# td-kwj-zp2023/webgpu-msm-twisted-edwards

Hardware: AMD Instinct MI355X
Metric: MSMs/sec at n=2^20 Twisted-Edwards BLS12 (pipelined throughput = 1000/ms_per_step; single-MSM latency in latency_ms) (higher is better)
Workload: dtype u32

## Files before the change

### webgpu-msm-twisted-edwards_amd/csrc/kernels.hip.hpp

```cpp
#pragma once
#include <hip/hip_runtime.h>
#include "curve.hpp"

namespace te {

#define TE_BATCH_MAX 8
struct batch_ptrs { const uint4* p[TE_BATCH_MAX]; };
struct batch_slabs { uint32_t s[TE_BATCH_MAX]; };

struct digits_params {
  uint32_t half[10];
  uint32_t zero_digit;
  uint32_t sc_stride;
  uint32_t n, nst;
  int num_windows;
  int w_first, w_step, nw_local;
  uint32_t half_code, logS, P, CH, chunk_len;
};

struct pnt_slot { uint4 q[8]; };
__device__ __forceinline__ void prep_points_block(uint32_t blk, uint4* __restrict__ lds, const uint4* __restrict__ pts, pnt_slot* __restrict__ recs, uint32_t n) {
  const uint32_t t = threadIdx.x, base = blk * 256u;
  const bool active = t < 256u;
  const uint32_t pieces_in = (n - base < 256u ? n - base : 256u) * 4u;
  const uint4* __restrict__ src = pts + (size_t)base * 4u;
  if (active) {
#pragma unroll
    for (int j = 0; j < 4; j++) {
      const uint32_t g = (uint32_t)j * 256u + t;
      lds[g] = src[g < pieces_in ? g : 0u];
    }
  }
  __syncthreads();
  uint4 a0 = make_uint4(0u, 0u, 0u, 0u), a1 = a0, b0 = a0, b1 = a0;
  if (active) { a0 = lds[4 * t + 0]; a1 = lds[4 * t + 1]; b0 = lds[4 * t + 2]; b1 = lds[4 * t + 3]; }
// ... 519 lines not shown
  __syncthreads();
  const uint32_t c0 = cnt_s[t];
  const size_t gb = (size_t)k * g.B + (size_t)p * g.S + t;
  if (!single) {
    if (c0) atomicAdd(&a.bucket_count[gb], c0);
    wait_own_accesses();
    __syncthreads();
    if (t == 0) pj[2] = (handoff_arrive(&a.part_ticket[k * g.P + p]) + 1u == (cntp + TE_L2_CAP - 1u) / TE_L2_CAP) ? 1u : 0u;
    __syncthreads();
    if (pj[2]) (void)seg_plan_block(p, k, t < g.S ? ld_agent(a.bucket_count + gb) : 0u, g, a.pa, PL, pb, cntp, sbp);
    return;
  }
  if (t < g.S) a.bucket_count[gb] = c0;
  const uint32_t ex = seg_plan_block(p, k, c0, g, a.pa, PL, pb, cntp, sbp);
  if (t < g.S) a.pa.bucket_cursor[gb] = pb + ex + c0;
  off_s[t] = ex;
  __syncthreads();
#pragma unroll
  for (int c = 0; c < 5; c++) {
    uint32_t kv[8], iv[8]; piece_group<PK>(r, c, kv, iv);
    const uint32_t e0 = ((uint32_t)c * 256u + t) * 8u;
#pragma unroll
    for (int e = 0; e < 8; e++) {
      const uint32_t pos = e0 + (uint32_t)e;
      if (pos >= head && pos < total) list[atomicAdd(&off_s[kv[e] & 0x7fffu], 1u)] = iv[e] | ((kv[e] >> 15) << 31);
    }
  }
  __syncthreads();
  uint32_t* out = a.sorted + (size_t)k * g.n + pb;
  for (uint32_t s = t; s < cntp; s += 256u) out[s] = list[s];
}

#define TE_ORDER_REGS 32u
__device__ __forceinline__ void order_scatter_block(uint32_t ob, uint32_t nob, uint32_t* __restrict__ lds, const uint32_t* __restrict__ lenv, uint32_t ids,
                                                    const uint32_t* __restrict__ size_hist, uint32_t* __restrict__ rel_cursor,
                                                    uint32_t* __restrict__ order, uint32_t* __restrict__ num_segments, uint32_t max_len) {
  uint32_t* const h = lds; uint32_t* const base = lds + 1024; uint32_t* const sm = lds + 2048;
  const uint32_t per = (ids + nob - 1) / nob;
  const uint32_t lo = min(ids, ob * per), hi = min(ids, lo + per);
  const bool in_regs = per <= TE_ORDER_REGS * 256u;
  uint32_t lv[TE_ORDER_REGS];
  if (in_regs) {
#pragma unroll
    for (uint32_t j = 0; j < TE_ORDER_REGS; j++) { const uint32_t g = lo + j * 256u + threadIdx.x; lv[j] = g < hi ? lenv[g] : TE_SEG_INVALID; }
  }
  for (uint32_t j = threadIdx.x; j < 1024u; j += 256u) h[j] = 0;
  {
    uint32_t run = 0;
    for (uint32_t c = (1023u - min(max_len, 1023u)) >> 8; c < 4u; c++) {
      const uint32_t s = 1023u - (c * 256u + threadIdx.x);
      uint32_t part[TE_HIST_COPIES];
#pragma unroll
      for (uint32_t r = 0; r < TE_HIST_COPIES; r++) part[r] = size_hist[r * 1024u + s];
      uint32_t cnt_s = 0;
#pragma unroll
      for (uint32_t r = 0; r < TE_HIST_COPIES; r++) cnt_s += part[r];
      uint32_t bt;
      const uint32_t ex = block_excl_scan(cnt_s, sm, bt);
      base[s] = run + ex;
      run += bt;
    }
    if (ob == 0 && threadIdx.x == 0) *num_segments = run;
  }
  __syncthreads();
  if (in_regs) {
#pragma unroll
    for (uint32_t j = 0; j < TE_ORDER_REGS; j++) if (lv[j] != TE_SEG_INVALID) atomicAdd(&h[min(lv[j], 1023u)], 1u);
  } else {
    for (uint32_t g = lo + threadIdx.x; g < hi; g += 256u) { const uint32_t l = lenv[g]; if (l != TE_SEG_INVALID) atomicAdd(&h[min(l, 1023u)], 1u); }
  }
  __syncthreads();
  for (uint32_t j = threadIdx.x; j < 1024u; j += 256u) { base[j] += h[j] ? atomicAdd(&rel_cursor[j], h[j]) : 0u; h[j] = 0; }
  __syncthreads();
  if (in_regs) {
#pragma unroll
    for (uint32_t j = 0; j < TE_ORDER_REGS; j++) {
      if (lv[j] == TE_SEG_INVALID) continue;
      const uint32_t sz = min(lv[j], 1023u);
      order[base[sz] + atomicAdd(&h[sz], 1u)] = lo + j * 256u + threadIdx.x;
    }
  } else {
    for (uint32_t g = lo + threadIdx.x; g < hi; g += 256u) {
      const uint32_t l = lenv[g];
      if (l == TE_SEG_INVALID) continue;
      const uint32_t sz = min(l, 1023u);
      order[base[sz] + atomicAdd(&h[sz], 1u)] = g;
    }
  }
}

#define TE_PLACE_LDS_WORDS (4u * 256u + TE_L2_LIST + TE_L2_LIST / 4u + 2u + 17u)
template <bool PK>
__device__ __forceinline__ void l2_place_piece(uint32_t p, uint32_t k, uint32_t a0, uint32_t b0, uint32_t* __restrict__ lds,
                                               const uint16_t* __restrict__ part_keys, const uint32_t* __restrict__ part_idx,
                                               uint32_t* __restrict__ bucket_cursor, uint32_t* __restrict__ sorted, const sort_geom& g) {
  uint32_t* const cnt_s = lds; uint32_t* const lex_s = lds + 256; uint32_t* const off_s = lds + 512; uint32_t* const gbase_s = lds + 768;
  uint32_t* const list = lds + 1024;
  uint8_t* const list_b = reinterpret_cast<uint8_t*>(list + TE_L2_LIST);
  uint32_t* const sm = list + TE_L2_LIST + TE_L2_LIST / 4u + 2u;
  const uint32_t t = threadIdx.x, len = b0 - a0;
  const uint16_t* keys_row = part_keys + (size_t)k * g.nst; const uint32_t* idx_row = part_idx + (size_t)k * g.nst;
  uint32_t* out = sorted + (size_t)k * g.n;
  cnt_s[t] = 0u;
  __syncthreads();
  piece_regs r; uint32_t head, total;
  load_piece<PK>(keys_row, idx_row, a0, b0, t, true, r, head, total);
#pragma unroll
  for (int c = 0; c < 5; c++) {
    uint32_t kv[8], iv[8]; piece_group<PK>(r, c, kv, iv);
    const uint32_t e0 = ((uint32_t)c * 256u + t) * 8u;
#pragma unroll
    for (int e = 0; e < 8; e++) { const uint32_t pos = e0 + (uint32_t)e; if (pos >= head && pos < total) atomicAdd(&cnt_s[kv[e] & 0x7fffu], 1u); }
  }
  __syncthreads();
  wave0_excl_scan(cnt_s, lex_s, 256u, &sm[16]);
  {
    const uint32_t c0 = cnt_s[t];
    gbase_s[t] = c0 ? atomicAdd(&bucket_cursor[(size_t)k * g.B + (size_t)p * g.S + t], c0) : 0u;
  }
  __syncthreads();
  off_s[t] = lex_s[t];
  gbase_s[t] -= lex_s[t];
  __syncthreads();
#pragma unroll
  for (int c = 0; c < 5; c++) {
    uint32_t kv[8], iv[8]; piece_group<PK>(r, c, kv, iv);
    const uint32_t e0 = ((uint32_t)c * 256u + t) * 8u;
#pragma unroll
    for (int e = 0; e < 8; e++) {
      const uint32_t pos = e0 + (uint32_t)e;
      if (pos >= head && pos < total) {
        const uint32_t b = kv[e] & 0x7fffu;
        const uint32_t slot = atomicAdd(&off_s[b], 1u);
        list[slot] = iv[e] | ((kv[e] >> 15) << 31); list_b[slot] = (uint8_t)b;
      }
    }
  }
  __syncthreads();
  for (uint32_t s = t; s < len; s += 256u) out[gbase_s[list_b[s]] + s] = list[s];
}

struct order_args { const uint32_t* lenv; uint32_t ids; const uint32_t* size_hist; uint32_t* rel_cursor; uint32_t* order; uint32_t* num_segments; uint32_t order_cols, max_len; };
template <bool PK>
__global__ void __launch_bounds__(256, TE_L2_WAVES) k_l2_place_order(const uint16_t* __restrict__ part_keys, const uint32_t* __restrict__ part_idx,
                                                           const uint32_t* __restrict__ part_start, const uint32_t* __restrict__ part_count,
                                                           uint32_t* __restrict__ bucket_cursor, uint32_t* __restrict__ sorted, sort_geom g, order_args oa) {
  __shared__ uint32_t lds[TE_PLACE_LDS_WORDS];
  if (blockIdx.x < oa.order_cols) {
    order_scatter_block(blockIdx.y * oa.order_cols + blockIdx.x, gridDim.y * oa.order_cols, lds, oa.lenv, oa.ids, oa.size_hist, oa.rel_cursor, oa.order, oa.num_segments, oa.max_len);
    return;
  }
  const uint32_t k = gridDim.y - 1u - blockIdx.y;
  const uint32_t px = blockIdx.x - oa.order_cols, extra = gridDim.x - oa.order_cols - g.P, bx = px < extra ? g.P + px : px - extra;
  const uint32_t* pc = part_count + k * g.P;
  uint32_t p, j;
  if (!l2_piece_of_block(bx, pc, g.P, bx < g.P ? 0u : part_count[gridDim.y * g.P + k], lds, lds + 32, p, j)) return;
  const uint32_t cntp = pc[p], pb = part_start[k * g.P + p];
  if (cntp <= TE_L2_CAP) return;
  const uint32_t a0 = pb + j * TE_L2_CAP;
  l2_place_piece<PK>(p, k, a0, min(pb + cntp, a0 + TE_L2_CAP), lds, part_keys, part_idx, bucket_cursor, sorted, g);
}

template <int N> struct geo {
  static constexpr uint32_t PW = 4u * N;
  static constexpr uint32_t PQ = PW / 4u;
  static constexpr uint32_t RW = N == 9 ? 27u : 4u * N;
  static constexpr uint32_t SQ = N == 9 ? 8u : N;
  static constexpr uint32_t LQ = (RW + 3u) / 4u;
};
template <int N> struct rec_slot { uint4 q[geo<N>::SQ]; };
static_assert(sizeof(rec_slot<9>) == sizeof(pnt_slot) && sizeof(rec_slot<14>) == 224, "record slots");

template <int N> __device__ __forceinline__ pnt_t<N> load_pnt(const rec_slot<N>* __restrict__ recs, uint32_t entry) {
  const uint4* q = recs[entry & 0x7fffffffu].q;
  constexpr uint32_t LQ = geo<N>::LQ;
  uint4 u[LQ];
#pragma unroll
  for (uint32_t j = 0; j < LQ; j++) u[j] = q[j];
  uint32_t w[4 * LQ];
#pragma unroll
  for (uint32_t j = 0; j < LQ; j++) { w[4 * j] = u[j].x; w[4 * j + 1] = u[j].y; w[4 * j + 2] = u[j].z; w[4 * j + 3] = u[j].w; }
  pnt_t<N> r;
// ... 47 lines not shown
#pragma unroll
  for (int j = 0; j < 10; j++) u[j] = reinterpret_cast<const u4a8*>(base)[j];
  const u2a8 t = *reinterpret_cast<const u2a8*>(base + 40);
  uint32_t w[42];
#pragma unroll
  for (int j = 0; j < 10; j++) { w[4 * j] = u[j].v[0]; w[4 * j + 1] = u[j].v[1]; w[4 * j + 2] = u[j].v[2]; w[4 * j + 3] = u[j].v[3]; }
  w[40] = t.v[0]; w[41] = t.v[1];
  pnt_aff377 r;
#pragma unroll
  for (int j = 0; j < 14; j++) { r.hm.v[j] = w[j]; r.hp.v[j] = w[14 + j]; r.dt.v[j] = w[28 + j]; }
  return r;
}
__device__ __forceinline__ void store_pnt_aff377(rec_aff377* dst, const pnt_aff377& r) {
#pragma unroll
  for (int j = 0; j < 14; j++) { dst->w[j] = r.hm.v[j]; dst->w[14 + j] = r.hp.v[j]; dst->w[28 + j] = r.dt.v[j]; }
}
template <int N, int RK> struct rec_kind;
template <int N> struct rec_kind<N, 0> {
  using slot = rec_slot<N>; using pnt = pnt_t<N>;
  static __device__ __forceinline__ pnt load(const slot* __restrict__ recs, uint32_t e) { return load_pnt<N>(recs, e); }
};
template <> struct rec_kind<14, 1> {
  using slot = rec_aff377; using pnt = pnt_aff377;
  static __device__ __forceinline__ pnt load(const slot* __restrict__ recs, uint32_t e) { return load_pnt_aff377(recs, e); }
};

struct __attribute__((aligned(4))) idx4 { uint32_t v[4]; };
#define TE_CLK_SLOTS 64u
#define TE_IDX_STRIP 16u
template <int N, int RK = 0>
__global__ void __launch_bounds__(256, N == 9 ? 3 : 2) k_accumulate(const typename rec_kind<N, RK>::slot* __restrict__ recs, const uint32_t* __restrict__ sorted,
                                                    const uint32_t* __restrict__ bucket_start, const uint32_t* __restrict__ bucket_count,
                                                    const uint32_t* __restrict__ seg_base, const uint32_t* __restrict__ seg_bucket,
                                                    const uint32_t* __restrict__ seg_lenv, const uint32_t* __restrict__ order,
                                                    const uint32_t* __restrict__ num_segments, ete_t<N>* __restrict__ buckets,
                                                    ete_t<N>* __restrict__ seg_out, uint32_t n, uint32_t logB, uint32_t seg_len, uint32_t ids, uint32_t onto,
                                                    uint32_t win_per_msm, batch_slabs slabs, unsigned long long* __restrict__ clk) {
  __shared__ uint32_t idx_strip[256 * TE_IDX_STRIP];
  using RT = rec_kind<N, RK>; using P = typename RT::pnt;
#if defined(TE_ACC_TWO_WAVES)
  if constexpr (N == 9) asm volatile("" ::: "v175");
#endif
  unsigned long long* const slot = clk ? clk + (blockIdx.x & (TE_CLK_SLOTS - 1u)) : nullptr;
  const unsigned long long t0_wall = clk ? (unsigned long long)wall_clock64() : 0ull, t0_core = clk ? (unsigned long long)clock64() : 0ull;
  if (clk && threadIdx.x == 0) atomicMax(slot, ~t0_wall);
  const uint32_t gid = blockIdx.x * 256u + threadIdx.x;
  if (gid >= (order ? *num_segments : ids)) return;
  const uint32_t sgm = order ? order[gid] : gid;
  const uint32_t g = seg_bucket[sgm];
  if (g == TE_SEG_INVALID) return;
  const uint32_t k = g >> logB;
  recs += (size_t)slabs.s[k / win_per_msm] * n;
  const uint32_t part = sgm - seg_base[g];
  const uint32_t cnt = seg_lenv[sgm];
  const uint32_t* lst = sorted + (size_t)k * n + bucket_start[g] + part * seg_len;
  ete_t<N> acc = (onto && part == 0u) ? load_ete<N>(buckets + g) : ete_identity_t<N>();
  if (cnt) {
    const uint32_t last = cnt - 1u;
    uint32_t j0 = 0;
    uint32_t e = lst[0], e_n = lst[min(1u, last)];
    P cur = RT::load(recs, e);
    if (!(onto && part == 0u)) {
      const P first = pnt_cneg(cur, (e >> 31) != 0u);
      e = e_n; e_n = lst[min(2u, last)];
      cur = RT::load(recs, e);
      acc = ete_from_pnt(first);
      j0 = 1;
    }
    uint32_t* const strip = idx_strip + threadIdx.x * TE_IDX_STRIP;
    auto refill = [&](uint32_t pos) {
      const idx4* src = reinterpret_cast<const idx4*>(lst + pos);
      idx4* dst = reinterpret_cast<idx4*>(strip);
#pragma unroll
      for (uint32_t h = 0; h < TE_IDX_STRIP / 4u; h += 2u) {
        const idx4 v0 = src[h], v1 = src[h + 1u];
        dst[h] = v0; dst[h + 1u] = v1;
      }
    };
    if (((j0 + 2u) & (TE_IDX_STRIP - 1u)) != 0u) refill((j0 + 2u) & ~(TE_IDX_STRIP - 1u));
    for (uint32_t j = j0; j < cnt; j++) {
      const uint32_t e_cur = e;
      P nxt = cur;
      const uint32_t pn = j + 2u;
      if ((pn & (TE_IDX_STRIP - 1u)) == 0u) refill(pn);
      const uint32_t e_nn = strip[pn & (TE_IDX_STRIP - 1u)];
      if (j + 1 < cnt) { e = e_n; nxt = RT::load(recs, e); }
      acc = ete_madd(acc, pnt_cneg(cur, (e_cur >> 31) != 0u));
      cur = nxt; e_n = e_nn;
    }
  }
  const bool whole = bucket_count[g] <= seg_len;
  store_ete<N>(whole ? buckets + g : seg_out + sgm, acc);
  if (clk && (uint32_t)__lane_id() == (uint32_t)__ffsll((long long)__ballot(1)) - 1u) {
    const unsigned long long t1_wall = (unsigned long long)wall_clock64(), t1_core = (unsigned long long)clock64();
    atomicMax(slot + TE_CLK_SLOTS, t1_wall);
    atomicAdd(slot + 2u * TE_CLK_SLOTS, t1_core - t0_core); atomicAdd(slot + 3u * TE_CLK_SLOTS, t1_wall - t0_wall);
  }
}

template <int N> struct sum_job_t {
  const ete_t<N>* in; ete_t<N>* out;
  uint32_t n_out;
  uint32_t K, inner;
  uint32_t in_per_window, out_per_window;
};
template <int N> struct sum_jobs_t { sum_job_t<N> j[4]; };
template <int N> __device__ __forceinline__ ete_t<N> pair_swap(const ete_t<N>& a) {
  ete_t<N> r;
#pragma unroll
  for (int i = 0; i < N; i++) {
    r.x.v[i] = (uint32_t)__builtin_amdgcn_mov_dpp((int)a.x.v[i], 0xb1, 0xf, 0xf, true);
    r.y.v[i] = (uint32_t)__builtin_amdgcn_mov_dpp((int)a.y.v[i], 0xb1, 0xf, 0xf, true);
    r.z.v[i] = (uint32_t)__builtin_amdgcn_mov_dpp((int)a.z.v[i], 0xb1, 0xf, 0xf, true);
    r.t.v[i] = (uint32_t)__builtin_amdgcn_mov_dpp((int)a.t.v[i], 0xb1, 0xf, 0xf, true);
  }
  return r;
}
template <int N, bool PAIR>
__global__ void __launch_bounds__(256, N == 9 ? 2 : 1) k_sum_groups(sum_jobs_t<N> js, uint32_t nw) {
  const sum_job_t<N>& j = js.j[blockIdx.y];
  constexpr uint32_t TPO = PAIR ? 2u : 1u;
  const uint32_t total = j.n_out * nw * TPO, Kt = j.K / TPO;
  for (uint32_t gt = blockIdx.x * 256u + threadIdx.x; gt < total; gt += gridDim.x * 256u) {
    const uint32_t g = gt / TPO, half = gt % TPO;
    const uint32_t k = g / j.n_out, o = g - k * j.n_out;
// ... 511 lines not shown
```

### webgpu-msm-twisted-edwards_amd/csrc/te_msm.hip

```cpp
#include <hip/hip_runtime.h>
#include <stdint.h>
#include <stdio.h>
#include <stdlib.h>
#include <string.h>
#include <string>
#include <vector>
#include <deque>
#include <algorithm>
#include <functional>
#include <chrono>
#include <thread>
#include <mutex>
#include <condition_variable>
#include <memory>
#if defined(__x86_64__)
#include <immintrin.h>
#endif

#include "../../include/te_msm.h"
#include "host_tail.hpp"
#include "synth.hpp"
#include "kernels.hip.hpp"
#include "check.hip.hpp"
#include "from_x.hip.hpp"
// ... 18 lines not shown
                                            : curve_sizes{TE_MSM_POINT_BYTES, TE_MSM_SCALAR_BYTES, sizeof(te::ete), sizeof(te::rec_slot<9>), TE_MSM_PARTIAL_BYTES, 64};
}
inline size_t rec_bytes_of(int curve, int rec_kind) { return (curve == TE_MSM_CURVE_BLS12_377_G1 && rec_kind == 1) ? sizeof(te::rec_aff377) : sizes_of(curve).rec; }
static_assert(TE377_TAIL_ROW_BYTES == TE_MSM_PARTIAL_BYTES_BLS12_377 && sizeof(te::ete_t<14>) * 5 == TE377_TAIL_ROW_BYTES, "row layout");
constexpr size_t TE_MAX_ROW_BYTES = TE377_TAIL_ROW_BYTES;

struct plan_t {
  int curve = 0;
  int c = 0, W = 0, nw = 0;
  int nw1 = 0, batch = 1;
  int w_first = 0, w_step = 1;
  uint32_t B = 0, logB = 0;
  int signed_digits = 1;
  uint32_t dw[4] = {0, 0, 0, 0};
  uint32_t CH = 0, chunk_len = 0, nst = 0;
  uint32_t seg_len = 64;
  uint32_t S = 0, logS = 0, P = 0;
  uint32_t packed = 0;
  int rec_kind = 0;
  int fb_rb = 0, fb_c = 0, fb_W = 0;
};

struct workset_t {
  hipStream_t stream = nullptr, copy_stream = nullptr;
  int hw_queue_class = -1;
  hipEvent_t ev_copy = nullptr, ev_start = nullptr;
  size_t cap[40] = {};
  uint8_t* d_recs = nullptr;
  uint16_t *d_digits = nullptr, *d_part_keys = nullptr;
  uint32_t *d_counts1 = nullptr, *d_part_start = nullptr, *d_part_count = nullptr, *d_part_idx = nullptr, *d_seg_part_base = nullptr;
  uint32_t *d_bucket_count = nullptr, *d_bucket_start = nullptr, *d_bucket_cursor = nullptr, *d_sorted = nullptr;
  uint32_t *d_seg_base = nullptr, *d_seg_bucket = nullptr, *d_seg_lenv = nullptr, *d_order = nullptr;
  uint32_t *d_split_list = nullptr, *d_chunk_list = nullptr;
  uint8_t *d_seg_out = nullptr, *d_buckets = nullptr, *d_red[4] = {};
  uint32_t *d_zero = nullptr; size_t zero_words = 0;
  size_t zero_clean_words = 0;
  uint32_t *d_err = nullptr, *d_num_seg = nullptr, *d_size_hist = nullptr, *d_size_cursor = nullptr;
  uint32_t* d_part_ticket = nullptr;
  uint8_t* d_partials = nullptr;
  uint32_t* h_err = nullptr;
  uint8_t* h_partials = nullptr;
  uint32_t* h_err_dev = nullptr;
  bool rows_on_host = false;
  hipEvent_t ev_done = nullptr;
  hipEvent_t ev_result = nullptr;
  hipEvent_t ev[ST_COUNT + 1] = {};
  plan_t plan; uint64_t n = 0; bool used = false;
  te_sched::slot_t slot;
  std::string job_err;
  int prof_level = 0;
  hipStream_t last_stream = nullptr;
  void *d_in_points = nullptr, *d_in_scalars = nullptr; size_t cap_in_points = 0, cap_in_scalars = 0;
  std::vector<hipEvent_t> piece_events;
  uint8_t* h_ring = nullptr; std::vector<hipEvent_t> ring_ev; size_t ring_next = 0;
  uint64_t idle_calls = 0;
  uint32_t* d_fb_remap = nullptr;
  uint32_t* d_fb_fill = nullptr;
  const void* fb_scalars = nullptr; uint64_t fb_n = 0;
  int slab = -1;
  bool slab_run = false;
  const uint8_t* recs_last = nullptr;
  te_bases* bound = nullptr;
  int pt_rc = 0; int64_t pt_index = -1; int pt_reason = 0;
  uint8_t* d_batch_rows = nullptr;
  uint32_t* d_in_idx = nullptr;
};
// ... 164 lines not shown

template <typename T> int ensure(te_ctx* ctx, workset_t& ws, T*& ptr, size_t& cap_bytes, size_t need_elems) {
  const size_t need = need_elems * sizeof(T);
  if (ptr && need <= cap_bytes) return 0;
  if (ptr) HIP_TRY(ctx, hipFree(ptr));
  ptr = nullptr; cap_bytes = 0;
  HIP_TRY(ctx, hipMalloc((void**)&ptr, need ? need : 16));
  cap_bytes = need;
  return 0;
}

int ensure_buffers(te_ctx* ctx, gpu_t& d, workset_t& ws, uint64_t n, const plan_t& p, bool need_recs = true) {
  HIP_TRY(ctx, hipSetDevice(d.device));
  const size_t nd = (size_t)p.nw * p.nst + 64, wb = (size_t)p.nw * p.B, ab = sizes_of(p.curve).acc;
  int rc = 0;
  if (need_recs && (rc = ensure(ctx, ws, ws.d_recs, ws.cap[0], (size_t)n * sizes_of(p.curve).rec * (size_t)p.batch))) return rc;
  if ((rc = ensure(ctx, ws, ws.d_digits, ws.cap[1], nd))) return rc;
  if ((rc = ensure(ctx, ws, ws.d_sorted, ws.cap[2], nd))) return rc;
  {
    const size_t c1 = (size_t)p.nw * p.CH * p.P;
    ws.zero_words = Z_END + c1 + wb + (size_t)p.nw * p.P + 64;
    { const uint32_t* before = ws.d_zero; if ((rc = ensure(ctx, ws, ws.d_zero, ws.cap[3], ws.zero_words))) return rc; if (ws.d_zero != before) ws.zero_clean_words = 0; }
    ws.d_err = ws.d_zero; ws.d_num_seg = ws.d_zero + Z_KEEP; ws.d_size_hist = ws.d_zero + Z_HIST; ws.d_size_cursor = ws.d_zero + Z_CURSOR;
    ws.d_partials = reinterpret_cast<uint8_t*>(ws.d_zero + Z_ROWS);
    ws.d_counts1 = ws.d_zero + Z_END; ws.d_bucket_count = ws.d_counts1 + c1; ws.d_part_ticket = ws.d_bucket_count + wb;
    ws.d_fb_fill = ws.d_part_ticket + (size_t)p.nw * p.P;
  }
  if (p.fb_rb && (rc = ensure(ctx, ws, ws.d_fb_remap, ws.cap[27], nd))) return rc;
  if ((rc = ensure(ctx, ws, ws.d_bucket_start, ws.cap[5], wb))) return rc;
  if ((rc = ensure(ctx, ws, ws.d_bucket_cursor, ws.cap[16], wb))) return rc;
  if ((rc = ensure(ctx, ws, ws.d_seg_part_base, ws.cap[17], (size_t)p.nw * p.P))) return rc;
  const size_t smax = wb + (size_t)p.nw * (n / (uint64_t)p.seg_len) + 16;
  if ((rc = ensure(ctx, ws, ws.d_order, ws.cap[7], smax))) return rc;
  if ((rc = ensure(ctx, ws, ws.d_seg_bucket, ws.cap[20], smax))) return rc;
  if ((rc = ensure(ctx, ws, ws.d_seg_lenv, ws.cap[21], smax))) return rc;
  if ((rc = ensure(ctx, ws, ws.d_seg_out, ws.cap[22], smax * ab))) return rc;
  if ((rc = ensure(ctx, ws, ws.d_seg_base, ws.cap[23], wb + 1))) return rc;
  if ((rc = ensure(ctx, ws, ws.d_split_list, ws.cap[24], wb + 1))) return rc;
  if ((rc = ensure(ctx, ws, ws.d_chunk_list, ws.cap[26], 2 * (wb + smax / TE_GIANT_RUN + 2)))) return rc;
  if ((rc = ensure(ctx, ws, ws.d_part_start, ws.cap[6], (size_t)p.nw * p.P))) return rc;
  if ((rc = ensure(ctx, ws, ws.d_buckets, ws.cap[8], wb * ab))) return rc;
  if ((rc = ensure(ctx, ws, ws.d_part_count, ws.cap[9], (size_t)p.nw * p.P + (size_t)p.nw))) return rc;
  if ((rc = ensure(ctx, ws, ws.d_part_keys, ws.cap[14], p.packed ? 8 : nd))) return rc;
  if ((rc = ensure(ctx, ws, ws.d_part_idx, ws.cap[15], nd))) return rc;
  if ((rc = ensure(ctx, ws, ws.d_red[0], ws.cap[10], (wb / 2 + 1) * ab))) return rc;
  if ((rc = ensure(ctx, ws, ws.d_red[1], ws.cap[11], (wb / 4 + 1) * ab))) return rc;
  if ((rc = ensure(ctx, ws, ws.d_red[2], ws.cap[12], (wb / 2 + 1) * ab))) return rc;
  if ((rc = ensure(ctx, ws, ws.d_red[3], ws.cap[13], (wb / 4 + 1) * ab))) return rc;
  return 0;
}

template <int C> void launch_digits(const te::batch_ptrs& sc, int batch, uint16_t* dg, const te::digits_params& prm, uint32_t* err, uint32_t* counts1, hipStream_t s) {
  hipLaunchKernelGGL(te::k_digits<C>, dim3((prm.nst + TE_DIG_BLOCK - 1u) / TE_DIG_BLOCK, batch), dim3(TE_DIG_THREADS), 0, s, sc, dg, prm, err, counts1);
}
static_assert(TE_BATCH_MAX == TE_MSM_MAX_BATCH, "batch tables");
template <int C> void launch_digits_ragged(const void* sc, const te::ragged_tab& tab, int batch, uint16_t* dg, const te::digits_params& prm, uint32_t* err, uint32_t* counts1, hipStream_t s) {
  hipLaunchKernelGGL(te::k_digits_ragged<C>, dim3((prm.nst + TE_DIG_BLOCK - 1u) / TE_DIG_BLOCK, batch), dim3(TE_DIG_THREADS), 0, s, static_cast<const uint4*>(sc), tab, dg, prm, err, counts1);
}
static_assert(TE_RAGGED_MAX == TE_BATCH_SEQ_MAX && TE_BATCH_SEQ_MAX == TE_MSM_BATCH_SEQ_MAX, "ragged tables");

struct msm_launch {
  te_ctx* ctx; workset_t& ws; plan_t p;
  const void* d_points; const void* d_scalars; uint64_t n; void* d_partials_out;
  int prof;
  hipStream_t stream;
  bool own_rows = false;
// ... 123 lines not shown
          const uint32_t per_row = (n32 + 511u) / 512u;
          hipLaunchKernelGGL(te::k_part_scatter_prep377, dim3(sblocks + rows * per_row), dim3(512), 0, stream, sa, sblocks, tab, row_slab,
                             reinterpret_cast<te::rec_slot<14>*>(recs_out()), n32, per_row, rows * per_row);
        } else {
          const uint32_t per_row = (n32 + 255u) / 256u;
          hipLaunchKernelGGL(te::k_part_scatter_prep, dim3(sblocks + rows * per_row), dim3(512), 0, stream, sa, sblocks, tab, row_slab,
                             reinterpret_cast<te::pnt_slot*>(recs_out()), n32, per_row, rows * per_row);
        }
      } else if (idx) {
        hipLaunchKernelGGL(te::k_part_scatter_indexed, dim3(p.CH, p.nw), dim3(512), 0, stream, sa, te::index_args{idx, idx_count, idx_pos, ws.d_err});
      } else {
        hipLaunchKernelGGL(te::k_part_scatter, dim3(p.CH, p.nw), dim3(512), 0, stream, sa);
      }
    }
    mark(ST_BSORT);
    if (p.nw > 0) {
      const uint32_t l2_blocks = p.P + n32 / TE_L2_CAP + 1u;
      te::l2_args la;
      la.part_keys = ws.d_part_keys; la.part_idx = ws.d_part_idx; la.part_start = ws.d_part_start; la.part_count = ws.d_part_count;
      la.bucket_count = ws.d_bucket_count; la.sorted = ws.d_sorted; la.part_ticket = ws.d_part_ticket; la.g = sg;
      la.pa.part_start = ws.d_part_start; la.pa.part_count = ws.d_part_count; la.pa.seg_part_base = ws.d_seg_part_base;
      la.pa.bucket_start = ws.d_bucket_start; la.pa.bucket_cursor = ws.d_bucket_cursor; la.pa.seg_base = ws.d_seg_base; la.pa.seg_bucket = ws.d_seg_bucket;
      la.pa.seg_lenv = ws.d_seg_lenv; la.pa.size_hist = ws.d_size_hist; la.pa.split_list = ws.d_split_list; la.pa.split_count = ws.d_num_seg + 1;
      la.pa.chunk_list = ws.d_chunk_list; la.pa.seg_len = p.seg_len; la.pa.cap_w = cap_w; la.pa.chunk_cap = chunk_cap();
      if (p.packed) hipLaunchKernelGGL(te::k_l2_local<true>, dim3(l2_blocks, p.nw), dim3(256), 0, stream, la);
      else hipLaunchKernelGGL(te::k_l2_local<false>, dim3(l2_blocks, p.nw), dim3(256), 0, stream, la);
      te::order_args oa;
      oa.lenv = ws.d_seg_lenv; oa.ids = smax(); oa.size_hist = ws.d_size_hist; oa.rel_cursor = ws.d_size_cursor; oa.order = ws.d_order; oa.num_segments = ws.d_num_seg;
      {
        const uint32_t by_regs = (smax() + TE_ORDER_REGS * 256u * (uint32_t)p.nw - 1u) / (TE_ORDER_REGS * 256u * (uint32_t)p.nw);
        oa.order_cols = std::min(64u, std::max(by_regs, (uint32_t)std::max(1, 128 / p.nw)));
      }
      oa.max_len = std::min(p.seg_len, 1023u);
      if (p.packed)
        hipLaunchKernelGGL(te::k_l2_place_order<true>, dim3(oa.order_cols + l2_blocks, p.nw), dim3(256), 0, stream, ws.d_part_keys, ws.d_part_idx, ws.d_part_start,
                           ws.d_part_count, ws.d_bucket_cursor, ws.d_sorted, sg, oa);
      else
        hipLaunchKernelGGL(te::k_l2_place_order<false>, dim3(oa.order_cols + l2_blocks, p.nw), dim3(256), 0, stream, ws.d_part_keys, ws.d_part_idx, ws.d_part_start,
                           ws.d_part_count, ws.d_bucket_cursor, ws.d_sorted, sg, oa);
    }
    mark(ST_ORDER);
    return 0;
  }

  bool bls() const { return p.curve == TE_MSM_CURVE_BLS12_377_G1; }

  template <int N, int RK> int accumulate_t() {
    mark(ST_ACCUM);
    if (p.nw > 0) {
      const uint32_t n32 = this->n32(), smax = this->smax();
      const uint32_t* order = ctx->opt_sort ? ws.d_order : nullptr;
      using slot_t = typename te::rec_kind<N, RK>::slot;
      hipLaunchKernelGGL((te::k_accumulate<N, RK>), dim3((smax + 255) / 256), dim3(256), 0, stream, reinterpret_cast<const slot_t*>(bound ? bound : recs_out()), ws.d_sorted,
                         ws.d_bucket_start, ws.d_bucket_count, ws.d_seg_base, ws.d_seg_bucket, ws.d_seg_lenv, order, ws.d_num_seg,
                         reinterpret_cast<te::ete_t<N>*>(ws.d_buckets), reinterpret_cast<te::ete_t<N>*>(ws.d_seg_out), n32, p.logB, p.seg_len, smax, onto ? 1u : 0u,
                         ragged ? (uint32_t)p.nw : (uint32_t)p.nw1, ragged ? te::batch_slabs{} : slabs(),
                         prof ? reinterpret_cast<unsigned long long*>(ws.d_zero + Z_CLOCK) : nullptr);
    }
    return 0;
  }
  int accumulate() { return bls() ? (p.rec_kind == 1 ? accumulate_t<14, 1>() : accumulate_t<14, 0>()) : accumulate_t<9, 0>(); }

  template <int N> int combine_t() {
    if (p.nw <= 0) return 0;
    using E = te::ete_t<N>;
    hipLaunchKernelGGL(te::k_seg_combine_all<N>, dim3(256 + 1024), dim3(256), 0, stream, ws.d_split_list, ws.d_num_seg + 1, ws.d_chunk_list,
                       ws.d_bucket_count, ws.d_seg_base, reinterpret_cast<E*>(ws.d_seg_out), reinterpret_cast<E*>(ws.d_buckets), p.seg_len, chunk_cap(), 256u,
                       ws.d_bucket_start, ws.d_bucket_cursor);
    return 0;
  }
  int combine() { return bls() ? combine_t<14>() : combine_t<9>(); }

  template <int N> int reduce_t() {
    if (p.nw > 0) {
      using E = te::ete_t<N>;
      const uint32_t w0 = p.dw[0], w1 = p.dw[1], w2 = p.dw[2], w3 = p.dw[3];
      const uint32_t L = 1u << (w0 + w1), H = 1u << (w2 + w3);
      struct chain_t { const E* cur; uint32_t n, r; E* buf[2]; int pp; };
      E* const bk = reinterpret_cast<E*>(ws.d_buckets);
      chain_t ch[2] = {{bk, p.B, L, {reinterpret_cast<E*>(ws.d_red[0]), reinterpret_cast<E*>(ws.d_red[1])}, 0},
                       {bk, p.B, H, {reinterpret_cast<E*>(ws.d_red[2]), reinterpret_cast<E*>(ws.d_red[3])}, 0}};
      for (;;) {
        te::sum_jobs_t<N> js; memset(&js, 0, sizeof js);
        uint32_t most = 0; int nj = 0;
        for (int i = 0; i < 2; i++) {
          chain_t& c = ch[i];
          if (c.r <= 4u) continue;
// ... 305 lines not shown
  HIP_TRY(ctx, hipEventRecord(ws.ev_done, stream));
  return 0;
}

int collect_stage_ms(te_ctx* ctx, const gpu_t& d, workset_t& ws) {
  if (!ws.prof_level) return 0;
  bool ok = true;
  for (int i = 0; i < ST_COUNT; i++) {
    float ms = -1.0f;
    if (ws.prof_level >= 2 || i == ST_ACCUM) ok = ok && hipEventElapsedTime(&ms, ws.ev[i], ws.ev[i + 1]) == hipSuccess;
    ctx->stage_ms[i] = ms;
  }
  {
    uint64_t raw[4 * TE_CLK_SLOTS]; memcpy(raw, ws.h_err + Z_CLOCK, sizeof raw);
    uint64_t c[4] = {0, 0, 0, 0};
    for (uint32_t i = 0; i < TE_CLK_SLOTS; i++) {
      c[0] = std::max(c[0], raw[i]); c[1] = std::max(c[1], raw[TE_CLK_SLOTS + i]);
      c[2] += raw[2 * TE_CLK_SLOTS + i]; c[3] += raw[3 * TE_CLK_SLOTS + i];
    }
    const int khz = d.wall_clock_khz;
    const bool have = c[0] && c[1] && khz > 0 && c[1] > ~c[0];
    const double ms = have ? (double)(c[1] - ~c[0]) / khz : -1.0;
    ctx->stage_ms[ST_COUNT] = (float)ms;
    ctx->stage_ms[ST_COUNT + 1] = (have && c[2] && c[3]) ? (float)((double)c[2] / (double)c[3] * khz * 1e-6) : -1.0f;
  }
  if (!ok) (void)hipGetLastError();
  ctx->have_stage_ms = ok;
  return 0;
}

void free_workset_buffers(workset_t& ws) {
  void** ptrs[] = {(void**)&ws.d_recs, (void**)&ws.d_digits, (void**)&ws.d_part_keys, (void**)&ws.d_zero, (void**)&ws.d_part_start, (void**)&ws.d_part_count,
                   (void**)&ws.d_part_idx, (void**)&ws.d_seg_part_base, (void**)&ws.d_bucket_start, (void**)&ws.d_bucket_cursor, (void**)&ws.d_sorted,
                   (void**)&ws.d_seg_base, (void**)&ws.d_seg_bucket, (void**)&ws.d_seg_lenv, (void**)&ws.d_order, (void**)&ws.d_split_list,
                   (void**)&ws.d_chunk_list, (void**)&ws.d_seg_out, (void**)&ws.d_buckets, (void**)&ws.d_red[0], (void**)&ws.d_red[1],
                   (void**)&ws.d_red[2], (void**)&ws.d_red[3], &ws.d_in_points, &ws.d_in_scalars, (void**)&ws.d_fb_remap, (void**)&ws.d_batch_rows, (void**)&ws.d_in_idx};
  for (void** q : ptrs) if (*q) { (void)hipFree(*q); *q = nullptr; }
  if (ws.h_ring) { (void)hipHostFree(ws.h_ring); ws.h_ring = nullptr; }
  memset(ws.cap, 0, sizeof ws.cap); ws.cap_in_points = ws.cap_in_scalars = 0;
  ws.zero_words = ws.zero_clean_words = 0;
  ws.d_err = ws.d_num_seg = ws.d_size_hist = ws.d_size_cursor = ws.d_counts1 = ws.d_bucket_count = ws.d_part_ticket = nullptr; ws.d_partials = nullptr;
  ws.used = false;
}

void free_dev(gpu_t& d) {
  (void)hipSetDevice(d.device);
  for (auto& sl : d.slabs) {
    if (sl.d) { (void)hipFree(sl.d); sl.d = nullptr; }
    for (hipEvent_t& e : sl.ev) if (e) { (void)hipEventDestroy(e); e = nullptr; }
    if (sl.conv_ev) { (void)hipEventDestroy(sl.conv_ev); sl.conv_ev = nullptr; }
  }
  d.slabs.clear();
  if (d.chk_stream) (void)hipStreamDestroy(d.chk_stream);
  if (d.chk_pts) (void)hipFree(d.chk_pts);
  if (d.chk_word) (void)hipFree(d.chk_word);
  if (d.chk_host) (void)hipHostFree(d.chk_host);
  d.chk_stream = nullptr; d.chk_pts = nullptr; d.chk_cap = 0; d.chk_word = d.chk_host = nullptr;
  if (d.h_batch_rows) (void)hipHostFree(d.h_batch_rows);
  d.h_batch_rows = nullptr; d.h_batch_cap = 0;
  for (workset_t& ws : d.ws) {
    free_workset_buffers(ws);
    if (ws.h_err) (void)hipHostFree(ws.h_err);
    for (hipEvent_t e : ws.ring_ev) if (e) (void)hipEventDestroy(e);
    if (ws.ev_done) (void)hipEventDestroy(ws.ev_done);
    if (ws.ev_result) (void)hipEventDestroy(ws.ev_result);
    for (auto& ev : ws.ev) if (ev) (void)hipEventDestroy(ev);
    if (ws.ev_copy) (void)hipEventDestroy(ws.ev_copy);
// ... 2239 lines not shown
  if (device_index < 0 || (size_t)device_index >= ctx->devs.size() || first > total || count > total - first) return set_err(ctx, TE_MSM_EINVAL, "bad arguments");
  if (record_bytes) *record_bytes = (int)bases->rec_bytes;
  uint64_t bytes = count * bases->rec_bytes;
  if (bytes > cap) bytes = cap;
  if (!bytes) return 0;
  HIP_TRY(ctx, hipSetDevice(ctx->devs[(size_t)device_index].device));
  HIP_TRY(ctx, hipMemcpy(dst, bases->recs[(size_t)device_index] + first * bases->rec_bytes, bytes, hipMemcpyDeviceToHost));
  return (int64_t)bytes;
}

int64_t te_msm_debug_read(te_ctx* ctx, const char* stage, void* dst, uint64_t cap) {
  device_guard restore_callers_device;
  if (!ctx || !stage || !dst) return TE_MSM_EINVAL;
  drain_workers(ctx);
  gpu_t& d = ctx->devs[0];
  workset_t& ws = d.ws[d.last_ws];
  if (!ws.used) return set_err(ctx, TE_MSM_ESTATE, "no run yet");
  const plan_t& p = ws.plan; const uint64_t n = ws.n;
  const void* src = nullptr; uint64_t bytes = 0;
  if (ws.zero_clean_words && (!strcmp(stage, "bucket_count") || !strcmp(stage, "num_segments") || !strcmp(stage, "partials")))
    return set_err(ctx, TE_MSM_ESTATE, "this stage lives in the block that is cleared behind an MSM's read-back: set option prezero = 0 before the run to keep it");
  if (!strcmp(stage, "records")) {
    if (!ws.recs_last) return set_err(ctx, TE_MSM_ESTATE, "the last run gathered from a bound point set: the work set holds no records of its own");
    src = ws.recs_last; bytes = n * sizes_of(p.curve).rec;
  }
  else if (!strcmp(stage, "digits")) { src = ws.d_digits; bytes = (uint64_t)p.nw * p.nst * 2; }
  else if (!strcmp(stage, "bucket_count")) { src = ws.d_bucket_count; bytes = (uint64_t)p.nw * p.B * 4; }
  else if (!strcmp(stage, "bucket_start")) { src = ws.d_bucket_start; bytes = (uint64_t)p.nw * p.B * 4; }
  else if (!strcmp(stage, "sorted")) { src = ws.d_sorted; bytes = (uint64_t)p.nw * n * 4; }
  else if (!strcmp(stage, "num_segments")) { src = ws.d_num_seg; bytes = 4; }
  else if (!strcmp(stage, "seg_bucket")) { src = ws.d_seg_bucket; bytes = ((uint64_t)p.nw * p.B + (uint64_t)p.nw * (n / p.seg_len)) * 4; }
  else if (!strcmp(stage, "seg_len")) { src = ws.d_seg_lenv; bytes = ((uint64_t)p.nw * p.B + (uint64_t)p.nw * (n / p.seg_len)) * 4; }
  else if (!strcmp(stage, "order")) { src = ws.d_order; bytes = ((uint64_t)p.nw * p.B + (uint64_t)p.nw * (n / p.seg_len)) * 4; }
  else if (!strcmp(stage, "part_start")) { src = ws.d_part_start; bytes = (uint64_t)p.nw * p.P * 4; }
  else if (!strcmp(stage, "part_count")) { src = ws.d_part_count; bytes = (uint64_t)p.nw * p.P * 4; }
  else if (!strcmp(stage, "part_keys") && !p.packed) { src = ws.d_part_keys; bytes = (uint64_t)p.nw * p.nst * 2; }
  else if (!strcmp(stage, "part_idx") && !p.packed) { src = ws.d_part_idx; bytes = (uint64_t)p.nw * p.nst * 4; }
  else if (!strcmp(stage, "part_keys") || !strcmp(stage, "part_idx")) {
    const bool want_keys = stage[5] == 'k';
    const uint64_t words = (uint64_t)p.nw * p.nst;
    std::vector<uint32_t> pk(words);
    HIP_TRY(ctx, hipSetDevice(d.device));
    HIP_TRY(ctx, hipDeviceSynchronize());
    HIP_TRY(ctx, hipMemcpy(pk.data(), ws.d_part_idx, words * 4, hipMemcpyDeviceToHost));
    uint64_t out_bytes = words * (want_keys ? 2 : 4);
    if (out_bytes > cap) out_bytes = cap;
    if (want_keys) { uint16_t* o = static_cast<uint16_t*>(dst); for (uint64_t i = 0; i < out_bytes / 2; i++) o[i] = (uint16_t)(((pk[i] >> 23) & 0xffu) | ((pk[i] >> 31) << 15)); }
    else { uint32_t* o = static_cast<uint32_t*>(dst); for (uint64_t i = 0; i < out_bytes / 4; i++) o[i] = pk[i] & 0x7fffffu; }
    return (int64_t)out_bytes;
  }
  else if (!strcmp(stage, "buckets")) { src = ws.d_buckets; bytes = (uint64_t)p.nw * p.B * sizes_of(p.curve).acc; }
  else if (!strcmp(stage, "partials")) { src = ws.d_partials; bytes = (uint64_t)p.W * sizes_of(p.curve).row; }
  else return set_err(ctx, TE_MSM_EINVAL, "unknown stage");
  if (bytes > cap) bytes = cap;
  HIP_TRY(ctx, hipSetDevice(d.device));
  HIP_TRY(ctx, hipDeviceSynchronize());
  HIP_TRY(ctx, hipMemcpy(dst, src, bytes, hipMemcpyDeviceToHost));
  return (int64_t)bytes;
}

}
```

Baseline: 1141.

## Precompute packed per-segment records in order scatter for accumulate kernel

The order-scatter stage now writes, for each sorted segment slot, a 16-byte record holding the row offset, count, first/whole flags, bucket and segment id, gathered from the seg_bucket, seg_base, bucket_start and bucket_count tables. The accumulate kernel reads one coalesced uint4 per thread instead of following order[] and then doing several dependent indirect loads. This removes a chain of scattered loads from the start of accumulate. In exchange the order stage does extra gathers and writes a larger buffer, and it loads the record before the bounds check, which relies on the padded allocation.

```diff
diff --git a/webgpu-msm-twisted-edwards_amd/csrc/kernels.hip.hpp b/webgpu-msm-twisted-edwards_amd/csrc/kernels.hip.hpp
--- a/webgpu-msm-twisted-edwards_amd/csrc/kernels.hip.hpp
+++ b/webgpu-msm-twisted-edwards_amd/csrc/kernels.hip.hpp
@@ -1,6 +1,7 @@
 #pragma once
 #include <hip/hip_runtime.h>
 #include "curve.hpp"
+#include "seg_record.hpp"
 
 namespace te {
 
@@ -586,9 +587,15 @@
 }
 
 #define TE_ORDER_REGS 32u
+#define TE_ORDER_REC_BATCH 16u
+struct seg_tables { const uint32_t *seg_bucket, *seg_base, *bucket_start, *bucket_count; uint4* seg_rec; uint32_t seg_len; };
+__device__ __forceinline__ uint4 seg_record_of(const seg_tables& st, uint32_t sgm, uint32_t g, uint32_t len, uint32_t sb, uint32_t bs, uint32_t bc) {
+  const te_seg::record r = te_seg::from_tables(sgm, g, len, sb, bs, bc, st.seg_len);
+  return make_uint4(r.w[0], r.w[1], r.w[2], r.w[3]);
+}
 __device__ __forceinline__ void order_scatter_block(uint32_t ob, uint32_t nob, uint32_t* __restrict__ lds, const uint32_t* __restrict__ lenv, uint32_t ids,
                                                     const uint32_t* __restrict__ size_hist, uint32_t* __restrict__ rel_cursor,
-                                                    uint32_t* __restrict__ order, uint32_t* __restrict__ num_segments, uint32_t max_len) {
+                                                    uint32_t* __restrict__ order, uint32_t* __restrict__ num_segments, uint32_t max_len, const seg_tables st) {
   uint32_t* const h = lds; uint32_t* const base = lds + 1024; uint32_t* const sm = lds + 2048;
   const uint32_t per = (ids + nob - 1) / nob;
   const uint32_t lo = min(ids, ob * per), hi = min(ids, lo + per);
@@ -598,6 +605,11 @@
 #pragma unroll
     for (uint32_t j = 0; j < TE_ORDER_REGS; j++) { const uint32_t g = lo + j * 256u + threadIdx.x; lv[j] = g < hi ? lenv[g] : TE_SEG_INVALID; }
   }
+  uint32_t gv[TE_ORDER_REGS];
+  if (in_regs) {
+#pragma unroll
+    for (uint32_t j = 0; j < TE_ORDER_REGS; j++) gv[j] = st.seg_bucket[min(lo + j * 256u + threadIdx.x, ids - 1u)];
+  }
   for (uint32_t j = threadIdx.x; j < 1024u; j += 256u) h[j] = 0;
   {
     uint32_t run = 0;
@@ -628,17 +640,31 @@
   __syncthreads();
   if (in_regs) {
 #pragma unroll
-    for (uint32_t j = 0; j < TE_ORDER_REGS; j++) {
-      if (lv[j] == TE_SEG_INVALID) continue;
-      const uint32_t sz = min(lv[j], 1023u);
-      order[base[sz] + atomicAdd(&h[sz], 1u)] = lo + j * 256u + threadIdx.x;
+    for (uint32_t j0 = 0; j0 < TE_ORDER_REGS; j0 += TE_ORDER_REC_BATCH) {
+      uint32_t sb[TE_ORDER_REC_BATCH], bs[TE_ORDER_REC_BATCH], bc[TE_ORDER_REC_BATCH];
+#pragma unroll
+      for (uint32_t u = 0; u < TE_ORDER_REC_BATCH; u++) {
+        const uint32_t g = lv[j0 + u] != TE_SEG_INVALID ? gv[j0 + u] : 0u;
+        sb[u] = st.seg_base[g]; bs[u] = st.bucket_start[g]; bc[u] = st.bucket_count[g];
+      }
+#pragma unroll
+      for (uint32_t u = 0; u < TE_ORDER_REC_BATCH; u++) {
+        const uint32_t j = j0 + u;
+        if (lv[j] == TE_SEG_INVALID) continue;
+        const uint32_t sz = min(lv[j], 1023u), sgm = lo + j * 256u + threadIdx.x;
+        const uint32_t pos = base[sz] + atomicAdd(&h[sz], 1u);
+        order[pos] = sgm;
+        st.seg_rec[pos] = seg_record_of(st, sgm, gv[j], lv[j], sb[u], bs[u], bc[u]);
+      }
     }
   } else {
-    for (uint32_t g = lo + threadIdx.x; g < hi; g += 256u) {
-      const uint32_t l = lenv[g];
+    for (uint32_t sgm = lo + threadIdx.x; sgm < hi; sgm += 256u) {
+      const uint32_t l = lenv[sgm];
       if (l == TE_SEG_INVALID) continue;
-      const uint32_t sz = min(l, 1023u);
-      order[base[sz] + atomicAdd(&h[sz], 1u)] = g;
+      const uint32_t sz = min(l, 1023u), g = st.seg_bucket[sgm];
+      const uint32_t pos = base[sz] + atomicAdd(&h[sz], 1u);
+      order[pos] = sgm;
+      st.seg_rec[pos] = seg_record_of(st, sgm, g, l, st.seg_base[g], st.bucket_start[g], st.bucket_count[g]);
     }
   }
 }
@@ -694,14 +720,14 @@
   for (uint32_t s = t; s < len; s += 256u) out[gbase_s[list_b[s]] + s] = list[s];
 }
 
-struct order_args { const uint32_t* lenv; uint32_t ids; const uint32_t* size_hist; uint32_t* rel_cursor; uint32_t* order; uint32_t* num_segments; uint32_t order_cols, max_len; };
+struct order_args { const uint32_t* lenv; uint32_t ids; const uint32_t* size_hist; uint32_t* rel_cursor; uint32_t* order; uint32_t* num_segments; uint32_t order_cols, max_len; seg_tables st; };
 template <bool PK>
 __global__ void __launch_bounds__(256, TE_L2_WAVES) k_l2_place_order(const uint16_t* __restrict__ part_keys, const uint32_t* __restrict__ part_idx,
                                                            const uint32_t* __restrict__ part_start, const uint32_t* __restrict__ part_count,
                                                            uint32_t* __restrict__ bucket_cursor, uint32_t* __restrict__ sorted, sort_geom g, order_args oa) {
   __shared__ uint32_t lds[TE_PLACE_LDS_WORDS];
   if (blockIdx.x < oa.order_cols) {
-    order_scatter_block(blockIdx.y * oa.order_cols + blockIdx.x, gridDim.y * oa.order_cols, lds, oa.lenv, oa.ids, oa.size_hist, oa.rel_cursor, oa.order, oa.num_segments, oa.max_len);
+    order_scatter_block(blockIdx.y * oa.order_cols + blockIdx.x, gridDim.y * oa.order_cols, lds, oa.lenv, oa.ids, oa.size_hist, oa.rel_cursor, oa.order, oa.num_segments, oa.max_len, oa.st);
     return;
   }
   const uint32_t k = gridDim.y - 1u - blockIdx.y;
@@ -815,7 +841,7 @@
 __global__ void __launch_bounds__(256, N == 9 ? 3 : 2) k_accumulate(const typename rec_kind<N, RK>::slot* __restrict__ recs, const uint32_t* __restrict__ sorted,
                                                     const uint32_t* __restrict__ bucket_start, const uint32_t* __restrict__ bucket_count,
                                                     const uint32_t* __restrict__ seg_base, const uint32_t* __restrict__ seg_bucket,
-                                                    const uint32_t* __restrict__ seg_lenv, const uint32_t* __restrict__ order,
+                                                    const uint32_t* __restrict__ seg_lenv, const uint4* __restrict__ seg_rec,
                                                     const uint32_t* __restrict__ num_segments, ete_t<N>* __restrict__ buckets,
                                                     ete_t<N>* __restrict__ seg_out, uint32_t n, uint32_t logB, uint32_t seg_len, uint32_t ids, uint32_t onto,
                                                     uint32_t win_per_msm, batch_slabs slabs, unsigned long long* __restrict__ clk) {
@@ -828,22 +854,30 @@
   const unsigned long long t0_wall = clk ? (unsigned long long)wall_clock64() : 0ull, t0_core = clk ? (unsigned long long)clock64() : 0ull;
   if (clk && threadIdx.x == 0) atomicMax(slot, ~t0_wall);
   const uint32_t gid = blockIdx.x * 256u + threadIdx.x;
-  if (gid >= (order ? *num_segments : ids)) return;
-  const uint32_t sgm = order ? order[gid] : gid;
-  const uint32_t g = seg_bucket[sgm];
-  if (g == TE_SEG_INVALID) return;
+  te_seg::fields f;
+  if (seg_rec) {
+    const uint4 r = seg_rec[gid];
+    if (gid >= *num_segments) return;
+    f = te_seg::unpack(te_seg::record{{r.x, r.y, r.z, r.w}});
+  } else {
+    if (gid >= ids) return;
+    const uint32_t gb = seg_bucket[gid];
+    if (gb == TE_SEG_INVALID) return;
+    f = te_seg::unpack(te_seg::from_tables(gid, gb, seg_lenv[gid], seg_base[gb], bucket_start[gb], bucket_count[gb], seg_len));
+  }
+  const uint32_t g = f.g, sgm = f.sgm, cnt = f.cnt;
   const uint32_t k = g >> logB;
   recs += (size_t)slabs.s[k / win_per_msm] * n;
-  const uint32_t part = sgm - seg_base[g];
-  const uint32_t cnt = seg_lenv[sgm];
-  const uint32_t* lst = sorted + (size_t)k * n + bucket_start[g] + part * seg_len;
-  ete_t<N> acc = (onto && part == 0u) ? load_ete<N>(buckets + g) : ete_identity_t<N>();
+  const uint64_t lst_word = (uint64_t)k * n + f.row_off;
+  const bool continues = onto && f.first;
+  ete_t<N> acc = continues ? load_ete<N>(buckets + g) : ete_identity_t<N>();
+  const uint32_t* lst = sorted + lst_word;
   if (cnt) {
     const uint32_t last = cnt - 1u;
     uint32_t j0 = 0;
     uint32_t e = lst[0], e_n = lst[min(1u, last)];
     P cur = RT::load(recs, e);
-    if (!(onto && part == 0u)) {
+    if (!continues) {
       const P first = pnt_cneg(cur, (e >> 31) != 0u);
       e = e_n; e_n = lst[min(2u, last)];
       cur = RT::load(recs, e);
@@ -872,8 +906,7 @@
       cur = nxt; e_n = e_nn;
     }
   }
-  const bool whole = bucket_count[g] <= seg_len;
-  store_ete<N>(whole ? buckets + g : seg_out + sgm, acc);
+  store_ete<N>(f.whole ? buckets + g : seg_out + sgm, acc);
   if (clk && (uint32_t)__lane_id() == (uint32_t)__ffsll((long long)__ballot(1)) - 1u) {
     const unsigned long long t1_wall = (unsigned long long)wall_clock64(), t1_core = (unsigned long long)clock64();
     atomicMax(slot + TE_CLK_SLOTS, t1_wall);
diff --git a/webgpu-msm-twisted-edwards_amd/csrc/seg_record.hpp b/webgpu-msm-twisted-edwards_amd/csrc/seg_record.hpp
--- /dev/null
+++ b/webgpu-msm-twisted-edwards_amd/csrc/seg_record.hpp
@@ -0,0 +1,36 @@
+#pragma once
+
+#include <stdint.h>
+
+#ifndef TE_HD
+#if defined(__HIPCC__)
+#include <hip/hip_runtime.h>
+#define TE_HD __host__ __device__ __forceinline__
+#else
+#define TE_HD inline
+#endif
+#endif
+
+namespace te_seg {
+
+struct record { uint32_t w[4]; };
+struct fields { uint32_t row_off, cnt, g, sgm; bool first, whole; };
+
+constexpr uint32_t kCntMask = (1u << 30) - 1u, kFirstBit = 1u << 30, kWholeBit = 1u << 31;
+
+TE_HD record pack(const fields& f) {
+  record r;
+  r.w[0] = f.row_off; r.w[1] = (f.cnt & kCntMask) | (f.first ? kFirstBit : 0u) | (f.whole ? kWholeBit : 0u); r.w[2] = f.g; r.w[3] = f.sgm;
+  return r;
+}
+TE_HD fields unpack(const record& r) {
+  fields f;
+  f.row_off = r.w[0]; f.cnt = r.w[1] & kCntMask; f.first = (r.w[1] & kFirstBit) != 0u; f.whole = (r.w[1] & kWholeBit) != 0u; f.g = r.w[2]; f.sgm = r.w[3];
+  return f;
+}
+TE_HD record from_tables(uint32_t sgm, uint32_t g, uint32_t len, uint32_t seg_base_g, uint32_t bucket_start_g, uint32_t bucket_count_g, uint32_t seg_len) {
+  const uint32_t part = sgm - seg_base_g;
+  return pack(fields{bucket_start_g + part * seg_len, len, g, sgm, part == 0u, bucket_count_g <= seg_len});
+}
+
+}
diff --git a/webgpu-msm-twisted-edwards_amd/csrc/te_msm.hip b/webgpu-msm-twisted-edwards_amd/csrc/te_msm.hip
--- a/webgpu-msm-twisted-edwards_amd/csrc/te_msm.hip
+++ b/webgpu-msm-twisted-edwards_amd/csrc/te_msm.hip
@@ -74,6 +74,7 @@
   uint32_t *d_bucket_count = nullptr, *d_bucket_start = nullptr, *d_bucket_cursor = nullptr, *d_sorted = nullptr;
   uint32_t *d_seg_base = nullptr, *d_seg_bucket = nullptr, *d_seg_lenv = nullptr, *d_order = nullptr;
   uint32_t *d_split_list = nullptr, *d_chunk_list = nullptr;
+  uint4* d_seg_rec = nullptr;
   uint8_t *d_seg_out = nullptr, *d_buckets = nullptr, *d_red[4] = {};
   uint32_t *d_zero = nullptr; size_t zero_words = 0;
   size_t zero_clean_words = 0;
@@ -304,6 +305,7 @@
   if ((rc = ensure(ctx, ws, ws.d_seg_part_base, ws.cap[17], (size_t)p.nw * p.P))) return rc;
   const size_t smax = wb + (size_t)p.nw * (n / (uint64_t)p.seg_len) + 16;
   if ((rc = ensure(ctx, ws, ws.d_order, ws.cap[7], smax))) return rc;
+  if ((rc = ensure(ctx, ws, ws.d_seg_rec, ws.cap[30], smax + 256))) return rc;
   if ((rc = ensure(ctx, ws, ws.d_seg_bucket, ws.cap[20], smax))) return rc;
   if ((rc = ensure(ctx, ws, ws.d_seg_lenv, ws.cap[21], smax))) return rc;
   if ((rc = ensure(ctx, ws, ws.d_seg_out, ws.cap[22], smax * ab))) return rc;
@@ -493,6 +495,7 @@
         oa.order_cols = std::min(64u, std::max(by_regs, (uint32_t)std::max(1, 128 / p.nw)));
       }
       oa.max_len = std::min(p.seg_len, 1023u);
+      oa.st = te::seg_tables{ws.d_seg_bucket, ws.d_seg_base, ws.d_bucket_start, ws.d_bucket_count, ws.d_seg_rec, p.seg_len};
       if (p.packed)
         hipLaunchKernelGGL(te::k_l2_place_order<true>, dim3(oa.order_cols + l2_blocks, p.nw), dim3(256), 0, stream, ws.d_part_keys, ws.d_part_idx, ws.d_part_start,
                            ws.d_part_count, ws.d_bucket_cursor, ws.d_sorted, sg, oa);
@@ -510,10 +513,10 @@
     mark(ST_ACCUM);
     if (p.nw > 0) {
       const uint32_t n32 = this->n32(), smax = this->smax();
-      const uint32_t* order = ctx->opt_sort ? ws.d_order : nullptr;
+      const uint4* seg_rec = ctx->opt_sort ? ws.d_seg_rec : nullptr;
       using slot_t = typename te::rec_kind<N, RK>::slot;
       hipLaunchKernelGGL((te::k_accumulate<N, RK>), dim3((smax + 255) / 256), dim3(256), 0, stream, reinterpret_cast<const slot_t*>(bound ? bound : recs_out()), ws.d_sorted,
-                         ws.d_bucket_start, ws.d_bucket_count, ws.d_seg_base, ws.d_seg_bucket, ws.d_seg_lenv, order, ws.d_num_seg,
+                         ws.d_bucket_start, ws.d_bucket_count, ws.d_seg_base, ws.d_seg_bucket, ws.d_seg_lenv, seg_rec, ws.d_num_seg,
                          reinterpret_cast<te::ete_t<N>*>(ws.d_buckets), reinterpret_cast<te::ete_t<N>*>(ws.d_seg_out), n32, p.logB, p.seg_len, smax, onto ? 1u : 0u,
                          ragged ? (uint32_t)p.nw : (uint32_t)p.nw1, ragged ? te::batch_slabs{} : slabs(),
                          prof ? reinterpret_cast<unsigned long long*>(ws.d_zero + Z_CLOCK) : nullptr);
@@ -885,7 +888,7 @@
 void free_workset_buffers(workset_t& ws) {
   void** ptrs[] = {(void**)&ws.d_recs, (void**)&ws.d_digits, (void**)&ws.d_part_keys, (void**)&ws.d_zero, (void**)&ws.d_part_start, (void**)&ws.d_part_count,
                    (void**)&ws.d_part_idx, (void**)&ws.d_seg_part_base, (void**)&ws.d_bucket_start, (void**)&ws.d_bucket_cursor, (void**)&ws.d_sorted,
-                   (void**)&ws.d_seg_base, (void**)&ws.d_seg_bucket, (void**)&ws.d_seg_lenv, (void**)&ws.d_order, (void**)&ws.d_split_list,
+                   (void**)&ws.d_seg_base, (void**)&ws.d_seg_bucket, (void**)&ws.d_seg_lenv, (void**)&ws.d_order, (void**)&ws.d_seg_rec, (void**)&ws.d_split_list,
                    (void**)&ws.d_chunk_list, (void**)&ws.d_seg_out, (void**)&ws.d_buckets, (void**)&ws.d_red[0], (void**)&ws.d_red[1],
                    (void**)&ws.d_red[2], (void**)&ws.d_red[3], &ws.d_in_points, &ws.d_in_scalars, (void**)&ws.d_fb_remap, (void**)&ws.d_batch_rows, (void**)&ws.d_in_idx};
   for (void** q : ptrs) if (*q) { (void)hipFree(*q); *q = nullptr; }
@@ -3191,6 +3194,7 @@
   else if (!strcmp(stage, "seg_bucket")) { src = ws.d_seg_bucket; bytes = ((uint64_t)p.nw * p.B + (uint64_t)p.nw * (n / p.seg_len)) * 4; }
   else if (!strcmp(stage, "seg_len")) { src = ws.d_seg_lenv; bytes = ((uint64_t)p.nw * p.B + (uint64_t)p.nw * (n / p.seg_len)) * 4; }
   else if (!strcmp(stage, "order")) { src = ws.d_order; bytes = ((uint64_t)p.nw * p.B + (uint64_t)p.nw * (n / p.seg_len)) * 4; }
+  else if (!strcmp(stage, "seg_records")) { src = ws.d_seg_rec; bytes = ((uint64_t)p.nw * p.B + (uint64_t)p.nw * (n / p.seg_len)) * 16; }
   else if (!strcmp(stage, "part_start")) { src = ws.d_part_start; bytes = (uint64_t)p.nw * p.P * 4; }
   else if (!strcmp(stage, "part_count")) { src = ws.d_part_count; bytes = (uint64_t)p.nw * p.P * 4; }
   else if (!strcmp(stage, "part_keys") && !p.packed) { src = ws.d_part_keys; bytes = (uint64_t)p.nw * p.nst * 2; }
```

Result: no change. 1146 (median of 3 runs) (+0.4%).
